# labicon/dp-ilqr

Hardware: AMD Instinct MI355X
Metric: ilqr_subproblems_per_sec (higher is better)
Workload: dtype f64; 1 GPU; cfg2: batches of 1024 independent 5-agent DoubleIntDynamics4D iLQR sub-problems per GPU per step, T=50, scripts/analysis.py scenario distribution, tol=1e-3, n_lqr_iter=50; 2468 steps = 2527232 distinct seeds per GPU, window of 6144 in flight; 1 repetition(s) of the job on disjoint seeds, the median is reported; batch_per_gpu=1024, window=6144, n_x=20, n_u=10, horizon=50, parallelism=single GPU

## Files before the change

### dpilqr_amd/csrc/admit_order.hpp

```cpp
#pragma once
#include <cstdint>

#if defined(__HIPCC__)
#include <hip/hip_runtime.h>
#define DPILQR_HD __host__ __device__
#else
#define DPILQR_HD
#endif

namespace dpilqr {

enum CostOrder : int { kOrderOff = 0, kOrderSpread = 1, kOrderGrouped = 2 };
constexpr int kDefaultCostOrder = kOrderSpread;

constexpr int kOrderMinLive = 1024;
constexpr int kOrderClasses = 64;

struct SweepDeal {
    int n, n_cus, waves, per_layer, layers, rounds, lo, extra;
    DPILQR_HD SweepDeal(int n_, int n_cus_, int waves_) : n(n_), n_cus(n_cus_), waves(waves_) {
        const int lpr = waves / 4;
        per_layer = 4 * n_cus;
        layers = (n + per_layer - 1) / per_layer;
        rounds = (layers + lpr - 1) / lpr;
        lo = rounds > 0 ? layers / rounds : 0;
        extra = rounds > 0 ? layers - lo * rounds : 0;
    }
    DPILQR_HD int layers_of(int round) const { return lo + (round < extra ? 1 : 0); }
    DPILQR_HD int first_layer(int round) const { return round * lo + (round < extra ? round : extra); }
    DPILQR_HD int round_of_layer(int layer) const {
        const int head = extra * (lo + 1);
        return layer < head ? layer / (lo + 1) : extra + (layer - head) / (lo > 0 ? lo : 1);
    }
    DPILQR_HD int slot(int round, int cu, int wave) const {
        if (round >= rounds || wave >= 4 * layers_of(round)) return -1;
        const int s = (first_layer(round) + (wave >> 2)) * per_layer + (wave & 3) * n_cus + cu;
        return s < n ? s : -1;
    }
};

DPILQR_HD inline int order_position(int rank, const SweepDeal& D, int order) {
    if (order != kOrderGrouped) return rank;
    const int round = D.round_of_layer(rank / D.per_layer);
    const int f = D.first_layer(round), m = D.layers_of(round);
    const int q = rank - f * D.per_layer;
    int base = 4 * m, e = 0;
    if (round == D.rounds - 1) {
        const int rem = D.n - (D.layers - 1) * D.per_layer;
        base = 4 * (m - 1) + rem / D.n_cus;
        e = rem % D.n_cus;
    }
    int cu, w;
    if (q < e * (base + 1)) { cu = q / (base + 1); w = q - cu * (base + 1); }
    else { const int q2 = q - e * (base + 1), per = base > 0 ? base : 1; cu = e + q2 / per; w = q2 - (cu - e) * per; }
    return (f + (w >> 2)) * D.per_layer + (w & 3) * D.n_cus + cu;
}

DPILQR_HD inline int order_class(int key, int T) {
    const int top = T + 1;
    const int c = top < kOrderClasses ? key : (int)((int64_t)key * (kOrderClasses - 1) / top);
    return c < 0 ? 0 : (c > kOrderClasses - 1 ? kOrderClasses - 1 : c);
}

#if defined(__HIPCC__) && defined(DPILQR_ADMIT_ORDER_KERNELS)

constexpr int kKeyStagedAgents = 5;
__global__ void __launch_bounds__(256) k_cost_keys(const double* __restrict__ X, const double* __restrict__ radius, int64_t radius_bstride,
                                                   const int32_t* __restrict__ list, const int32_t* __restrict__ count, int B, int T, int k,
                                                   int min_live, int32_t* __restrict__ key) {
    __shared__ double2 sP[4][64 * kKeyStagedAgents];
    const int n = count ? *count : B;
    if (n <= min_live) return;
    const int wave = (int)threadIdx.x >> 6, lane = threadIdx.x & 63;
    const int pos = (int)blockIdx.x * 4 + wave;
    if (pos >= n) return;
    const int b = list ? list[pos] : pos;
    if (b < 0 || b >= B) return;
    const double r = radius[(int64_t)b * radius_bstride];
    const double lim = r * r * (1.0 + 1e-12);
    const int nx = 4 * k;
    const double* Xb = X + (int64_t)b * (T + 1) * nx;
    const bool staged = k <= kKeyStagedAgents;
    int cnt = 0;
    for (int t0 = 0; t0 <= T; t0 += 64) {
        const int rows = min(64, T + 1 - t0);
        bool near = false;
        if (staged) {
            const double2* src = reinterpret_cast<const double2*>(Xb + (int64_t)t0 * nx);
            for (int e = lane; e < rows * k; e += 64) sP[wave][e] = src[2 * e];
            __builtin_amdgcn_wave_barrier();
            asm volatile("" ::: "memory");
            if (lane < rows) {
                double2 p[kKeyStagedAgents];
#pragma unroll
                for (int i = 0; i < kKeyStagedAgents; ++i) p[i] = sP[wave][lane * k + min(i, k - 1)];
#pragma unroll
                for (int i = 0; i < kKeyStagedAgents; ++i)
#pragma unroll
                    for (int j = i + 1; j < kKeyStagedAgents; ++j) {
                        const double ddx = p[i].x - p[j].x, ddy = p[i].y - p[j].y;
                        const double s2 = ddx * ddx + ddy * ddy;
                        near = near || (j < k && !(s2 > lim));
                    }
            }
            __builtin_amdgcn_wave_barrier();
            asm volatile("" ::: "memory");
        } else if (lane < rows) {
            const double* row = Xb + (int64_t)(t0 + lane) * nx;
            for (int i = 0; i < k; ++i)
                for (int j = i + 1; j < k; ++j) {
                    const double ddx = row[4 * i] - row[4 * j], ddy = row[4 * i + 1] - row[4 * j + 1];
                    const double s2 = ddx * ddx + ddy * ddy;
                    near = near || !(s2 > lim);
                }
        }
        cnt += __popcll(__builtin_amdgcn_ballot_w64(near));
    }
    if (lane == 0) key[pos] = cnt;
}

__global__ void __launch_bounds__(1024) k_order_list(const int32_t* __restrict__ src, int32_t* __restrict__ dst, const int32_t* __restrict__ count,
                                                     const int32_t* __restrict__ key, int T, int n_cus, int waves, int order, int min_live) {
    static_assert(kOrderClasses == 64, "the prefix sums below are one wavefront's, a bin per lane");
    __shared__ int hist[kOrderClasses], cursor[kOrderClasses];
    const int n = *count;
    if (n <= min_live || order == kOrderOff) {
        for (int i = threadIdx.x; i < n; i += blockDim.x) dst[i] = src[i];
        return;
    }
    if (threadIdx.x < kOrderClasses) hist[threadIdx.x] = 0;
    __syncthreads();
    for (int i = threadIdx.x; i < n; i += blockDim.x) atomicAdd(&hist[kOrderClasses - 1 - order_class(key[i], T)], 1);
    __syncthreads();
    if (threadIdx.x < kOrderClasses) {
        const int own = hist[threadIdx.x];
        int run = own;
        for (int off = 1; off < kOrderClasses; off <<= 1) {
            const int below = __shfl_up(run, off);
            if ((int)threadIdx.x >= off) run += below;
        }
        cursor[threadIdx.x] = run - own;
    }
    __syncthreads();
    const SweepDeal deal(n, n_cus, waves);
    for (int i = threadIdx.x; i < n; i += blockDim.x) {
        const int rank = atomicAdd(&cursor[kOrderClasses - 1 - order_class(key[i], T)], 1);
        const int pos = order_position(rank, deal, order);
        if (pos >= 0 && pos < n) dst[pos] = src[i];
    }
}

// ... 4 lines not shown
```

### dpilqr_amd/csrc/dpilqr_hip.hip

```cpp
#include <hip/hip_runtime.h>

#include <cstdarg>
#include <cstdio>
#include <algorithm>
#include <cstdlib>
#include <cstring>
#include <new>
#include <vector>

#include "dpilqr_hip.h"
#include "admit_order.hpp"
#include "launch.hpp"
#include "models.hpp"
#include "tiles.hpp"

namespace dpilqr {

static thread_local char g_err[512] = "";

int32_t fail(int32_t code, const char* fmt, ...) {
    va_list ap;
    va_start(ap, fmt);
    vsnprintf(g_err, sizeof(g_err), fmt, ap);
    va_end(ap);
// ... 368 lines not shown
    };

    int32_t* admitted_dev = counts + kCountRing;
    S.fault = counts + kCountRing + 1;
    static const bool no_static = route_flag("DPILQR_TILES_NO_STATIC");
    const int um = hint_model(D);
    const bool fused = sh.fused;
    const bool static_part = !fused && !sh.big && !no_static && D.R_bstride == 0 &&
                             (um == kDoubleInt4D || um == kDoubleInt6D || um == kHumanLin6D);
    if (!resume) {
        double a[DPILQR_N_ALPHA];
        alpha_table(a);
        const int init_n = D.B > kCountRing + 2 ? D.B : kCountRing + 2;
        hipLaunchKernelGGL(k_init_state, dim3((init_n + 255) / 256), dim3(256), 0, st, D.B, S.mu, S.delta, status, n_bwd, n_fwd,
                           singular, counts, kCountRing + 2, alphas, a[0], a[1], a[2], a[3], a[4], a[5], a[6], a[7], a[8], a[9]);
        HIP_TRY(hipGetLastError());
        prof.begin(3, -1, st);
        rc = Passes<R>::forward(D, kModeRollout, x0, X, U, nullptr, nullptr, nullptr, 1, nullptr, nullptr, S.J_star, S, nullptr,
                                nullptr, D.B, st);
        if (rc) return bail(rc);
        prof.end(st);
        hipLaunchKernelGGL(k_copy_f64, dim3((D.B + 255) / 256), dim3(256), 0, st, D.B, S.J_star, S.J_last);
        if (n_lqr_iter > 0) {
            if (!fused && hipMemsetAsync(tiles, 0, W.K - W.tiles, st) != hipSuccess) return bail(fail(DPILQR_EHIP, "hipMemsetAsync failed"));
            if (static_part) {
                if constexpr (sizeof(R) == 8) {
                    if ((rc = launch_make_tiles(D, X, U, tiles, nullptr, nullptr, Wn, true, false, st))) return bail(rc);
                }
            }
        }
    }

    static const int order_route = route_flag("DPILQR_NO_COST_ORDER") ? (int)kOrderOff : route_int("DPILQR_COST_ORDER", kDefaultCostOrder);
    const int order = (sizeof(R) == 8 && fused && (order_route == kOrderSpread || order_route == kOrderGrouped)) ? order_route : (int)kOrderOff;
    int32_t* keys = reinterpret_cast<int32_t*>(ws + W.Xc);
    int surv = 0;
    size_t n_iterations = 0;
    auto enqueue_iteration = [&](int it, int upper) -> int32_t {
        int32_t* cur = lists + (size_t)surv * Wn;
        int32_t* other = lists + (size_t)(surv ^ 1) * Wn;
        int32_t* cur_n = counts + (it % kCountRing);
        int32_t* nxt_n = counts + ((it + 1) % kCountRing);
        int32_t* mail = solver ? solver->dev + kMailWords * (it % kMailRing) : nullptr;
        hipLaunchKernelGGL(k_admit, dim3(1), dim3(256), 0, st, cur, cur_n, nxt_n, admitted_dev, D.B, Wn, mail,
                           (solver && solver->progress) ? 1 : 0, t_admit, S.fault);
        if (solver) HIP_TRY(hipEventRecord(solver->ev[it % kMailRing], st));
        int32_t r = DPILQR_OK;
        const int order_waves = order ? fused_sweep_tier(D, upper) : 0;
        if (order_waves > 0) {
            if constexpr (sizeof(R) == 8) {
                if ((r = launch_cost_keys(D, X, cur, cur_n, upper, kOrderMinLive, keys, st))) return r;
                if ((r = launch_order_list(cur, other, cur_n, keys, D.T, device_cus(), order_waves, order, kOrderMinLive, st))) return r;
            }
            S.next_items = cur;
            cur = other;
        } else {
            S.next_items = other;
            surv ^= 1;
        }
        S.next_count = nxt_n;
        if (fused) {
            if constexpr (sizeof(R) == 8) {
                prof.begin(1, it, st);
                if ((r = launch_riccati_fused(D, X, U, S.mu, K, d, singular, cur, cur_n, upper, S.gains_by_item, st))) return r;
                prof.end(st, g_sweep_waves);
            }
        } else if (!sh.big) {
            if constexpr (sizeof(R) == 8) {
                prof.begin(0, it, st);
                if ((r = launch_make_tiles(D, X, U, tiles, cur, cur_n, upper, true, static_part, st))) return r;
                prof.end(st);
                prof.begin(1, it, st);
                if ((r = launch_riccati(D.B, D.T, n, m, tiles, S.mu, K, d, singular, cur, cur_n, upper, S.gains_by_item, D.n_s,
                                        D.n_c, st)))
                    return r;
                prof.end(st, g_sweep_waves);
            }
        } else {
            prof.begin(1, it, st);
            if ((r = Passes<R>::sweep_big(D, X, U, S.mu, K, d, singular, cur, cur_n, upper, S.gains_by_item, tiles, st))) return r;
            prof.end(st, 0);
        }
        prof.begin(2, it, st);
        if ((r = Passes<R>::forward(D, kModeLineSearch, nullptr, X, U, K, d, alphas, DPILQR_N_ALPHA, Xc, Uc, nullptr, S, cur, cur_n,
// ... 416 lines not shown
                               float* K_out, float* d_out, void* stream) {
    if (!solver) {
        const int32_t rc = default_solver(&solver);
        if (rc) return rc;
    }
    return solve_impl<float>(solver, desc, x0, U, n_lqr_iter, tol, t_kill, window, workspace, workspace_bytes, X, J, status, n_bwd,
                             n_fwd, trace, K_out, d_out, 0, 0, as_stream(stream));
}
int32_t dpilqr_solve_enqueue(const dpilqr_batch_desc* desc, const double* x0, double* U, int32_t n_lqr_iter, double tol,
                             double t_kill, int32_t window, void* workspace, int64_t workspace_bytes, double* X, double* J, int32_t* status,
                             int32_t* n_bwd, int32_t* n_fwd, double* trace, double* K_out, double* d_out,
                             int32_t n_global_iter, int32_t resume, void* stream) {
    return solve_impl<double>(nullptr, desc, x0, U, n_lqr_iter, tol, t_kill, window, workspace, workspace_bytes, X, J, status, n_bwd,
                              n_fwd, trace, K_out, d_out, n_global_iter, resume, as_stream(stream));
}
int64_t dpilqr_solve_iterations_bound(const dpilqr_batch_desc* desc, int32_t window, int32_t n_lqr_iter) {
    if (!desc || desc->B < 0 || n_lqr_iter < 0) return fail(DPILQR_EINVAL, "solve_iterations_bound: bad argument");
    const int64_t W = window_of(*desc, window);
    return ((int64_t)desc->B + W - 1) / W * n_lqr_iter + 1;
}

int32_t dpilqr_debug_stamps(void* buf) {
    int32_t rc = set_stamp_buffer_riccati(buf);
    return rc ? rc : set_stamp_buffer_forward(buf);
}

int32_t dpilqr_cost_keys(const dpilqr_batch_desc* desc, const double* X, const int32_t* items, const int32_t* n_items, int32_t* keys,
                         void* stream) {
    int32_t rc = check_desc(desc);
    if (rc) return rc;
    if (desc->n_s != 4) return fail(DPILQR_EUNSUPPORTED, "cost_keys: n_s=%d, the keys are defined for the four-state family", desc->n_s);
    if (desc->B == 0) return DPILQR_OK;
    if (!X || !keys || ((items == nullptr) != (n_items == nullptr))) return fail(DPILQR_EINVAL, "cost_keys: NULL pointer");
    return launch_cost_keys(*desc, X, items, n_items, desc->B, -1, keys, as_stream(stream));
}

int32_t dpilqr_order_list(const int32_t* items, const int32_t* n_items, const int32_t* keys, int32_t T, int32_t n_cus, int32_t waves,
                          int32_t order, int32_t* out, void* stream) {
    if (!items || !n_items || !keys || !out) return fail(DPILQR_EINVAL, "order_list: NULL pointer");
    if (T < 1 || n_cus < 1 || (waves != 4 && waves != 8 && waves != 12) || (order != kOrderSpread && order != kOrderGrouped))
        return fail(DPILQR_EINVAL, "order_list: T=%d n_cus=%d waves=%d order=%d", T, n_cus, waves, order);
    return launch_order_list(items, out, n_items, keys, T, n_cus, waves, order, -1, as_stream(stream));
}

int32_t dpilqr_order_position(int32_t rank, int32_t n, int32_t n_cus, int32_t waves, int32_t order) {
    if (n < 1 || rank < 0 || rank >= n || n_cus < 1 || (waves != 4 && waves != 8 && waves != 12) ||
        (order != kOrderSpread && order != kOrderGrouped))
        return fail(DPILQR_EINVAL, "order_position: rank=%d n=%d n_cus=%d waves=%d order=%d", rank, n, n_cus, waves, order);
    return order_position(rank, SweepDeal(n, n_cus, waves), order);
}

int32_t dpilqr_profile_enable(dpilqr_solver* solver, int32_t enable) {
    Profiler& g_prof = solver ? solver->prof : g_default_solver.prof;
    const int32_t prev = g_prof.on ? 1 : 0;
    g_prof.on = (enable & 1) != 0;
    g_prof.mask = (enable >> 1) & 0xF ? (enable >> 1) & 0xF : 0xF;
    return prev;
}

int32_t dpilqr_profile_read(dpilqr_solver* solver, double ms[4], int64_t launches[4], int64_t items[4], int32_t reset) {
    if (!ms || !launches || !items) return fail(DPILQR_EINVAL, "profile_read: NULL pointer");
    Profiler& g_prof = solver ? solver->prof : g_default_solver.prof;
    for (int c = 0; c < 4; ++c) {
        ms[c] = g_prof.ms[c]; launches[c] = g_prof.launches[c]; items[c] = g_prof.items[c];
        if (reset) { g_prof.ms[c] = 0; g_prof.launches[c] = 0; g_prof.items[c] = 0; }
    }
    return DPILQR_OK;
// ... 21 lines not shown
```

### dpilqr_amd/csrc/launch.hpp

```cpp
#pragma once
#include <hip/hip_runtime.h>

#include <cstdint>
#include <cstdlib>

#include "dpilqr_hip.h"
#include "solve_state.hpp"

namespace dpilqr {

int32_t fail(int32_t code, const char* fmt, ...);
const char* last_error();

#define HIP_TRY(expr)                                                                                 \
    do {                                                                                              \
        hipError_t e_ = (expr);                                                                       \
        if (e_ != hipSuccess) return ::dpilqr::fail(DPILQR_EHIP, "%s failed: %s", #expr, hipGetErrorString(e_)); \
    } while (0)

constexpr int kMaxLds = 160 * 1024;

template <typename Kern>
inline int32_t allow_lds(Kern kern, size_t bytes) {
    if (bytes > (size_t)kMaxLds) return fail(DPILQR_EUNSUPPORTED, "needs %zu B of LDS per workgroup (> %d)", bytes, kMaxLds);
// ... 78 lines not shown
    return grid_items <= cus ? grid_items : (grid_items + cus * wv - 1) / (cus * wv) * cus;
}
inline int sweep_max_waves() { static const int v = route_int("DPILQR_MFMA_WAVES", 12); return v; }
template <typename Kern, typename... Args>
int32_t launch_sweep_kernel(Kern kern, int wv, int threads, size_t lds, int grid_items, int cus, hipStream_t st, const Args&... args) {
    const int32_t rc = allow_lds(kern, lds);
    if (rc) return rc;
    hipLaunchKernelGGL(kern, dim3(sweep_grid(grid_items, cus, wv)), dim3(threads), lds, st, args...);
    HIP_TRY(hipGetLastError());
    g_sweep_waves = wv;
    return DPILQR_OK;
}
template <typename T> struct same_type { using type = T; };
template <typename Kern, typename... Args>
int32_t launch_wave_sweep(Kern k4, typename same_type<Kern>::type k8, typename same_type<Kern>::type k12, size_t lds_per_wave,
                          int grid_items, int cus, hipStream_t st, const Args&... args) {
    const int wv = sweep_waves(grid_items, sweep_max_waves(), lds_per_wave, k12 != nullptr);
    return launch_sweep_kernel(wv == 12 ? k12 : (wv == 8 ? k8 : k4), wv, 64 * wv, lds_per_wave * wv, grid_items, cus, st, args...);
}
int32_t launch_riccati_team(const dpilqr_batch_desc& D, const double* X, const double* U, const double* mu, double* K, double* d,
                            int32_t* singular, const int32_t* items, const int32_t* n_items, int grid_items, int gains_by_item,
                            hipStream_t st);

int32_t launch_riccati_inprod(const dpilqr_batch_desc& D, const double* X, const double* U, const double* mu, double* K, double* d,
                              int32_t* singular, const int32_t* items, const int32_t* n_items, int grid_items, int gains_by_item,
                              hipStream_t st);

int32_t launch_riccati_bike(const dpilqr_batch_desc& D, const double* X, const double* U, const double* mu, double* K, double* d,
                            int32_t* singular, const int32_t* items, const int32_t* n_items, int grid_items, int gains_by_item,
                            hipStream_t st);

int fused_sweep_tier(const dpilqr_batch_desc& D, int grid_items);
int32_t launch_cost_keys(const dpilqr_batch_desc& D, const double* X, const int32_t* list, const int32_t* count, int grid_items,
                         int min_live, int32_t* key, hipStream_t st);
int32_t launch_order_list(const int32_t* src, int32_t* dst, const int32_t* count, const int32_t* key, int T, int cus, int waves,
                          int order, int min_live, hipStream_t st);

int32_t launch_linesearch_team(const dpilqr_batch_desc& D, double* X, double* U, const double* K, const double* d,
                               const double* alphas, double* Xc, double* Uc, const SolveState& S, const int32_t* items,
                               const int32_t* n_items, int grid_items, hipStream_t st);

int32_t launch_forward(const dpilqr_batch_desc& D, int mode, const double* x0, double* X, double* U, const double* K,
                       const double* d, const double* alphas, int ngrp, double* Xc, double* Uc, double* Jc,
                       const SolveState& S, const int32_t* items, const int32_t* n_items, int grid_items,
                       hipStream_t st);
int32_t set_stamp_buffer_forward(void* device_buffer);
int32_t launch_model_op(int op, int32_t n, int32_t ns, const int32_t* model, const double* x, const double* u, double dt,
                        double* o1, double* o2, hipStream_t st);
int32_t launch_cost_eval(const dpilqr_batch_desc& D, int32_t n_pts, const double* x, const double* u, int32_t terminal,
                         double* cost, hipStream_t st);
int32_t launch_pairwise_graph(int32_t S, int32_t N, int32_t k, int32_t n_s, const double* X, const double* radius,
                              int32_t* adj, hipStream_t st);


int32_t launch_policy_rollout(const dpilqr_batch_desc& D, const double* X, const double* U, const double* K, int32_t n_samples,
                              const double* x0s, const double* W, const double* u_lim, double* Xs, double* Us, double* J,
                              double* min_sep, double* goal_dist, hipStream_t st);
int32_t launch_policy_rollout_dec(const dpilqr_batch_desc& D, const double* X, const double* U_ff, const double* Kc, int32_t kc_max,
                                  const uint64_t* nbr_bits, int32_t n_samples, const double* x0s, const double* W, const double* u_lim,
                                  double* Xs, double* Us, double* J, double* min_sep, double* goal_dist, hipStream_t st);

int32_t launch_policy_rollout_dec_team(const dpilqr_batch_desc& D, const double* X, const double* U_ff, const double* Kc, int32_t kc_max,
                                       const uint64_t* nbr_bits, int32_t n_samples, const double* x0s, const double* W,
                                       const double* u_lim, double* Xs, double* Us, double* J, double* min_sep, double* goal_dist,
                                       hipStream_t st);

int32_t launch_policy_advance(const dpilqr_batch_desc& D, const double* X, const double* U, const double* K, int32_t kc_max,
// ... 38 lines not shown
```

### dpilqr_amd/csrc/riccati_mfma.hpp

```cpp
#pragma once
#include <hip/hip_runtime.h>

#include <type_traits>

#include "tiles.hpp"
#include "wave_util.hpp"

namespace dpilqr {

typedef double v4d __attribute__((ext_vector_type(4)));

template <int N, int M, int FUSED = 0, bool HELP = false>
struct MfmaCfg {
    static constexpr int NM = N + M;
    static constexpr int NP = N + 1;
    static constexpr int MK = round_up(M, 4);
    static constexpr int LAB = round_up(NM, 2);
    static constexpr int LT = LAB;
    static constexpr int LP = round_up(NP, 2);
    static constexpr int LQ = LP;
    static constexpr int LG = round_up(M + NP, 2);
    static constexpr int LK = LP;
    static constexpr int LM = N;
    static constexpr int KROWS = MK + 2;
// ... 182 lines not shown
#pragma unroll
                for (int q = 0; q < 3; ++q)
                    if (r0 + q < M) { tm[q] = v[r0 + q] * ninv; asm volatile("" : "+v"(tm[q])); }
                if (r0 + 2 >= M) asm volatile("s_nop 1");
#pragma unroll
                for (int q = 0; q < 3; ++q)
                    if (r0 + q < M) { v[r0 + q] = fmac_row_nn(v[r0 + q], tm[q], v[kk], kk); asm volatile("" : "+v"(v[r0 + q])); }
            }
            }
        } else {
#pragma unroll
            for (int r = kk + 1; r < M; ++r) {
                const double l = readlane_f64(v[r], kk) * inv;
                v[r] = fma(-l, v[kk], v[r]);
            }
        }
    }
#pragma unroll
    for (int r = 0; r < M; ++r) v_io[r] = v[r];
}

__device__ __forceinline__ void wave_barrier_all() { asm volatile("s_waitcnt lgkmcnt(0)\n\ts_barrier" ::: "memory"); }

template <bool ON>
__device__ __forceinline__ int phase_lane(int lane) {
    if constexpr (ON) asm volatile("" : "+v"(lane));
    return lane;
}

struct FusedArgs {
    dpilqr_batch_desc D;
    const double* X;
    const double* U;
};

template <int N, int M, int WAVES, int NS, int NC, int FUSED, bool PAD = false, bool HELP = false, int PNS = 0>
__device__ __forceinline__ void riccati_mfma_sweep(
    int B, int T, const double* __restrict__ tiles, const double* __restrict__ mu_arr, double* __restrict__ Kout,
    double* __restrict__ dout, int32_t* __restrict__ singular, const int32_t* __restrict__ items,
    const int32_t* __restrict__ n_items, int gains_by_item, int n_cus, FusedArgs F, int n_rec = N, int m_rec = M) {
    using C = MfmaCfg<N, M, FUSED, HELP>;
    static_assert(!FUSED || (NS == 4 && NC == 2), "the fused variants are written for the four-state family's blocks");
    static_assert(!HELP || (FUSED != 0 && WAVES == 4), "the helper wavefront serves the fused forms at one item per SIMD");
    static_assert(!PAD || (NS == 0 && FUSED == 0), "padding while loading is written for the dense record-fed form");
    static_assert(PNS == 0 || (NS == 0 && FUSED == 0 && !HELP), "in-sweep production builds on the dense form (padded, or of the exact size: n_rec = N, m_rec = M)");
    constexpr bool INP = PNS > 0;
    using IC = InprodCfg<N, M, PNS>;
    constexpr bool FGEN = (FUSED == 2);
    constexpr int NM = C::NM, NP = C::NP, MK = C::MK, LAB = C::LAB, LT = C::LT, LP = C::LP, LQ = C::LQ, LG = C::LG;
    constexpr int LK = C::LK, LM = C::LM, T_NM = C::T_NM, T_NP = C::T_NP, T_N = C::T_N, T_M = C::T_M;
    const int wave_all = threadIdx.x >> 6;
    const bool helper = HELP && wave_all >= 4;
    const int wave = HELP ? (wave_all & 3) : wave_all;
    const int n = n_items ? *n_items : B;
    constexpr int LPR = WAVES / 4;
    const int per_layer = 4 * n_cus;
    const int layers = (n + per_layer - 1) / per_layer;
    const int rounds = (layers + LPR - 1) / LPR;
    const int round = (int)blockIdx.x / n_cus, cu = (int)blockIdx.x - round * n_cus;
    if (round >= rounds) return;
    const int lo = layers / rounds, extra = layers - lo * rounds;
    const int my_layers = lo + (round < extra ? 1 : 0);
    const int first_layer = round * lo + min(round, extra);
    if (wave >= 4 * my_layers) return;
    const int slot = (first_layer + (wave >> 2)) * per_layer + (wave & 3) * n_cus + cu;
    if (slot >= n) return;
// ... 51 lines not shown
            wave_barrier_all();
            {
                t_cur = T - 1;
#include "riccati_mfma_lane.inc"
                fused_prefetch(T - 1);
            }
            for (int t = T - 1; t >= 0; --t) {
                t_cur = t;
#include "riccati_mfma_lane.inc"
                __builtin_amdgcn_s_waitcnt(0x0F70);
                fused_step_data(t, nullptr);
                if (lane == 0) sFflag[0] = f_prox ? 1.0 : 0.0;
                if (t > 0) fused_prefetch(t - 1);
                if constexpr (C::TEAM_TAIL) {
                    if (t < T - 1) {
                        wave_barrier_all();
                        constexpr int IT = 1;
#include "riccati_mfma_team_tail.inc"
                    }
                }
                wave_barrier_all();
            }
            if constexpr (C::TEAM_TAIL) {
                t_cur = 0;
#include "riccati_mfma_lane.inc"
                wave_barrier_all();
                constexpr int IT = 1;
#include "riccati_mfma_team_tail.inc"
                wave_barrier_all();
            }
            return;
        }
    }
    if constexpr (FUSED) {
        const ItemParams IP = item_params(F.D, b);
        constexpr int FKA_ = C::F_KA;
        const int ag_ = min(lane0 / LPA, KA - 1), sub2_ = min(lane0 - (lane0 / LPA) * LPA, (NM - 1) / RPL);
#pragma unroll
        for (int r = 0; r < RPL; ++r) {
#pragma unroll
            for (int c = 0; c < NSC; ++c) lvc[r][c] = 0.0;
            lv_h[r] = -1; lv_neg[r] = false;
            const int ip = min(RPL * sub2_ + r, NM - 1);
            if (ip < N) {
                const int ar = ip >> 2, li = ip & 3;
                if (ar == ag_) {
                    const double* Qa = IP.Q + (FGEN ? 16 * ag_ : 0);
#pragma unroll
                    for (int c = 0; c < NS; ++c) lvc[r][c] = F.D.w_ref * (Qa[li * 4 + c] + Qa[c * 4 + li]);
                }
                if (FKA_ > 1 && li < 2) {
                    lv_neg[r] = ar != ag_;
                    lv_h[r] = (ar == ag_) ? (C::oFD - C::oFH) + ag_ * 4 + li * 2
                                          : ((ar < ag_) ? pair_index(ar, ag_, FKA_) : pair_index(ag_, ar, FKA_)) * 4 + li * 2;
                }
            } else {
                const int a = ip - N;
                if ((a >> 1) == ag_) {
                    const double* Ra = IP.R + (FGEN ? 4 * ag_ : 0);
                    lvc[r][NS] = F.D.w_ref * (Ra[(a & 1) * 2] + Ra[a & 1]);
                    lvc[r][NS + 1] = F.D.w_ref * (Ra[(a & 1) * 2 + 1] + Ra[2 + (a & 1)]);
                }
            }
        }
    }
#include "riccati_mfma_inprod.inc"
    {
    const int lane = lane0;
    for (int e = lane; e < C::total + IC::total; e += 64) lds[e] = 0.0;
    DPILQR_LDS_FENCE();
    if constexpr (INP) {
        inp_constants();
        inp_prefetch(T);
        inp_produce(T, true);
        for (int e = lane; e < N * N; e += 64) {
            const int i = e / N, j = e - i * N;
            sP[i * LP + j] = sLxx[e];
        }
        for (int i = lane; i < N; i += 64) sP[i * LP + N] = sLxu[i];
        DPILQR_LDS_FENCE();
        inp_lxx_blocks(false, true);
        inp_prefetch(T - 1);
    } else if constexpr (!FUSED) {
        const double* rec = base + (int64_t)T * L.stride;
        for (int e = lane; e < N * N; e += 64) {
            const int i = e / N, j = e - i * N;
            if constexpr (PAD) {
                const double val = rec[L.oLxx + min(i, n_rec - 1) * n_rec + min(j, n_rec - 1)];
                sP[i * LP + j] = (i < n_rec && j < n_rec) ? val : 0.0;
            } else {
            sP[i * LP + j] = rec[L.oLxx + e];
            }
        }
        for (int i = lane; i < N; i += 64) {
            const double val = rec[L.oLx + (PAD ? min(i, n_rec - 1) : i)];
            sP[i * LP + N] = (!PAD || i < n_rec) ? val : 0.0;
        }
    }
// ... 22 lines not shown
        fused_step_data(T, IP.Qf);
        for (int e = lane; e < N * N; e += 64) {
            const int i = e / N, j = e - i * N, ai = i >> 2, li = i & 3, aj = j >> 2, lj = j & 3;
            double val = 0.0;
            if (ai == aj) {
                const double* Qfa = IP.Qf + (FGEN ? 16 * ai : 0);
                val = F.D.w_ref * (Qfa[li * 4 + lj] + Qfa[lj * 4 + li]);
            }
            if (FKA > 1 && li < 2 && lj < 2 && f_prox) {
                double acc = 0.0;
                if (ai == aj) acc = sFD[ai * 4 + li * 2 + lj];
                else acc += -sFH[((ai < aj) ? pair_index(ai, aj, FKA) : pair_index(aj, ai, FKA)) * 4 + li * 2 + lj];
                val += F.D.w_prox * acc;
            }
            sP[i * LP + j] = val;
        }
        for (int j = lane; j < N; j += 64) sP[j * LP + N] = sFL[j];
        DPILQR_LDS_FENCE();
        if constexpr (!HELP) fused_prefetch(T - 1);
    } else if constexpr (INP) {
    } else {
    prefetch_ab(T - 1);
    if constexpr (BD) {
        prefetch_bd_x(T - 1);
        if constexpr (!LATE_L) prefetch_bd_l(T - 1);
    } else {
        prefetch_lxu(T - 1);
        prefetch_l(T - 1);
    }
    }
    __builtin_amdgcn_s_waitcnt(0x0F70);
    }

#ifdef DPILQR_PHASE_STAMPS
    unsigned long long ph[8] = {0, 0, 0, 0, 0, 0, 0, 0}, ph_t = __builtin_amdgcn_s_memtime();
#define MPHASE(i) { asm volatile("s_waitcnt lgkmcnt(0)" ::: "memory"); const unsigned long long now_ = __builtin_amdgcn_s_memtime(); ph[i] += now_ - ph_t; ph_t = now_; }
#elif defined(DPILQR_PHASE_MARKS)
#define MPHASE(i) asm volatile("; ==== end of phase " #i);
#else
#define MPHASE(i)
#endif
    for (int t = T - 1; t >= 0; --t) {
        const int tn = t > 0 ? t - 1 : 0;
        t_cur = t;
        {
        const int lane = phase_lane<REMAT>(lane0);
#include "riccati_mfma_lane.inc"
        if constexpr (HELP) {
            wave_barrier_all();
            f_prox = __builtin_amdgcn_readfirstlane((int)(sFflag[0] != 0.0)) != 0;
        } else if constexpr (FUSED) {
            fused_step_data(t, nullptr);
            fused_prefetch(tn);
        } else if constexpr (INP) {
            inp_produce(t, false);
            inp_prefetch(tn);
        } else {
#pragma unroll
        for (int q = 0; q < C::AB_ROUNDS; ++q) *reinterpret_cast<v2d*>(ab_dst[q]) = nAB[q];
        DPILQR_LDS_FENCE();
        if constexpr (LATE_L) prefetch_bd_l(t);
        prefetch_ab(tn);
        }
        MPHASE(0)

        __builtin_amdgcn_s_setprio(1);
        if constexpr (FUSED) {
            const double fdt = F.D.dt;
            double acc[NSC][CPL], pr[NS][CPL];
#pragma unroll
            for (int l = 0; l < NS; ++l) {
                const v2d v = *reinterpret_cast<const v2d*>(bP + l * LP);
                pr[l][0] = v.x; pr[l][1] = v.y;
            }
            double fa[4] = {0.0, 0.0, 0.0, 0.0};
// ... 427 lines not shown
```

### dpilqr_amd/csrc/tu_order.hip

```cpp
#include <hip/hip_runtime.h>

#define DPILQR_ADMIT_ORDER_KERNELS
#include "admit_order.hpp"
#include "launch.hpp"
#include "riccati_mfma.hpp"

namespace dpilqr {

int fused_sweep_tier(const dpilqr_batch_desc& D, int grid_items) {
    if (!fused_wavefront_sweep_applies(D) || grid_items <= kOrderMinLive) return 0;
    const int n = D.k * D.n_s, m = D.k * D.n_c;
#define DPILQR_TIER(NN, MM) \
    if (n == NN && m == MM) return sweep_waves(grid_items, sweep_max_waves(), sizeof(double) * MfmaCfg<NN, MM, true>::total, true);
    DPILQR_TIER(4, 2) DPILQR_TIER(8, 4) DPILQR_TIER(12, 6) DPILQR_TIER(16, 8) DPILQR_TIER(20, 10)
#undef DPILQR_TIER
    return 0;
}

int32_t launch_cost_keys(const dpilqr_batch_desc& D, const double* X, const int32_t* list, const int32_t* count, int grid_items,
                         int min_live, int32_t* key, hipStream_t st) {
    if (grid_items <= 0) return DPILQR_OK;
    hipLaunchKernelGGL(k_cost_keys, dim3((grid_items + 3) / 4), dim3(256), 0, st, X, D.radius, D.radius_bstride, list, count, D.B, D.T,
                       D.k, min_live, key);
    HIP_TRY(hipGetLastError());
    return DPILQR_OK;
}

int32_t launch_order_list(const int32_t* src, int32_t* dst, const int32_t* count, const int32_t* key, int T, int cus, int waves,
                          int order, int min_live, hipStream_t st) {
    hipLaunchKernelGGL(k_order_list, dim3(1), dim3(1024), 0, st, src, dst, count, key, T, cus, waves, order, min_live);
    HIP_TRY(hipGetLastError());
    return DPILQR_OK;
}

}
```

### dpilqr_amd/csrc/tu_riccati.hip

```cpp
#include <hip/hip_runtime.h>

#include <cstdlib>
#include <cstring>

#include "launch.hpp"
#include "riccati.hpp"
#include "riccati_mfma.hpp"
#include "riccati_wg.hpp"

namespace dpilqr {

static int riccati_threads(int n) { return n <= 24 ? 64 : (n <= 36 ? 128 : 256); }

#define DPILQR_WAVE_SIZES(X) X(4, 2) X(8, 4) X(12, 6) X(16, 8) X(20, 10)

#define DPILQR_WG_SIZES(X)                                                                                      \
    X(6, 4, 2) X(7, 4, 2) X(8, 4, 2) X(9, 4, 2) X(10, 4, 2) X(11, 4, 2) X(12, 4, 2) X(13, 4, 2) X(14, 4, 2) X(15, 4, 2) \
    X(2, 6, 3) X(3, 6, 3) X(4, 6, 3) X(5, 6, 3) X(6, 6, 3) X(7, 6, 3) X(8, 6, 3) X(9, 6, 3) X(10, 6, 3)
#define DPILQR_WG_RECORD_SIZES(X) \
    X(2, 12, 4) X(3, 12, 4) X(4, 12, 4) X(5, 12, 4) X(1, 6, 3) X(1, 12, 4) X(2, 3, 2) X(4, 3, 2) X(6, 3, 2)

thread_local int g_sweep_waves = 0;

template <bool FUSED, typename... Args>
// ... 62 lines not shown
        DPILQR_TRY_PAD(24, 12)
#undef DPILQR_TRY_PAD
    }
    static const bool no_wg = route_flag("DPILQR_RICCATI_NO_WG");
    if (!generic && !no_wg && block_ns > 0) {
        const int32_t rc_w = launch_riccati_wg<false>(n, m, block_ns, block_nc, grid_items, st, B, T, tiles, mu, K, d, singular,
                                                      items, n_items, gains_by_item, FusedArgs{});
        if (rc_w != DPILQR_EUNSUPPORTED) return rc_w;
    }
    const size_t lds = riccati_lds_bytes(n, m);
    int32_t rc = allow_lds(k_riccati_generic, lds);
    if (rc) return rc;
    hipLaunchKernelGGL(k_riccati_generic, dim3(grid_items), dim3(riccati_threads(n)), lds, st, B, T, n, m, tiles, mu, K,
                       d, singular, items, n_items, gains_by_item);
    HIP_TRY(hipGetLastError());
    return DPILQR_OK;
}

int32_t launch_riccati_fused(const dpilqr_batch_desc& D, const double* X, const double* U, const double* mu, double* K,
                             double* d, int32_t* singular, const int32_t* items, const int32_t* n_items, int grid_items,
                             int gains_by_item, hipStream_t st) {
    g_sweep_waves = 0;
    if (grid_items <= 0) return DPILQR_OK;
    const int n = D.k * D.n_s, m = D.k * D.n_c;
    {
        const int32_t rc_ip = launch_riccati_inprod(D, X, U, mu, K, d, singular, items, n_items, grid_items, gains_by_item, st);
        if (rc_ip != DPILQR_EUNSUPPORTED) return rc_ip;
    }
    if (grid_items <= 1024 && sweep_max_waves() >= 4 && (fused_wavefront_sweep_applies(D) || fused_wavefront_general_applies(D))) {
        const int32_t rc_team = launch_riccati_team(D, X, U, mu, K, d, singular, items, n_items, grid_items, gains_by_item, st);
        if (rc_team != DPILQR_EUNSUPPORTED) return rc_team;
    }
    const int cus = device_cus();
#define DPILQR_TRY_FUSED(NN, MM)                                                                                   \
    if (n == NN && m == MM)                                                                                        \
        return launch_wave_sweep(k_riccati_mfma<NN, MM, 4, 4, 2, true>, k_riccati_mfma<NN, MM, 8, 4, 2, true>,     \
                                 k_riccati_mfma<NN, MM, 12, 4, 2, true>, sizeof(double) * MfmaCfg<NN, MM, true>::total, \
                                 grid_items, cus, st, D.B, D.T, nullptr, mu, K, d, singular, items, n_items, gains_by_item, \
                                 cus, FusedArgs{D, X, U});
    if (fused_wavefront_sweep_applies(D)) {
        DPILQR_WAVE_SIZES(DPILQR_TRY_FUSED)
    }
#undef DPILQR_TRY_FUSED
#define DPILQR_TRY_FUSED2(NN, MM)                                                                                  \
    if (n == NN && m == MM)                                                                                        \
        return launch_wave_sweep(k_riccati_mfma_general<NN, MM, 4>, k_riccati_mfma_general<NN, MM, 8>, nullptr,    \
                                 sizeof(double) * MfmaCfg<NN, MM, 2>::total, grid_items, cus, st, D.B, D.T, mu, K, d, \
                                 singular, items, n_items, gains_by_item, cus, FusedArgs{D, X, U});
    if (fused_wavefront_general_applies(D)) {
        DPILQR_WAVE_SIZES(DPILQR_TRY_FUSED2)
    }
#undef DPILQR_TRY_FUSED2
    if (fused_workgroup_sweep_applies(D))
        return launch_riccati_wg<true>(n, m, D.n_s, D.n_c, grid_items, st, D.B, D.T, nullptr, mu, K, d, singular, items, n_items,
                                       gains_by_item, FusedArgs{D, X, U});
    return DPILQR_EUNSUPPORTED;
}

int32_t set_stamp_buffer_riccati(void* buf) {
    void* p = buf;
    HIP_TRY(hipMemcpyToSymbol(HIP_SYMBOL(g_stamp_buf), &p, sizeof(p)));
    return DPILQR_OK;
}

}
```

Baseline: 1.080 million subproblems/s.

## Add decoupled per-agent Riccati prologue for trailing steps without proximity coupling

Adds a prologue to the fused MFMA Riccati sweep. While no proximity cost is active, it runs the backward recursion for the trailing timesteps with a cheap per-agent decoupled 4x2 block update and writes the gains directly. It drops to the full coupled MFMA loop at the first step with coupling or a failed conditioning check. The cost-order key also changes from a near-step count to the index of the last dense step, which matches the new per-item cost. The price is extra code, LDS traffic and divergence in the kernel, plus a different ordering heuristic.

```diff
diff --git a/dpilqr_amd/csrc/admit_order.hpp b/dpilqr_amd/csrc/admit_order.hpp
--- a/dpilqr_amd/csrc/admit_order.hpp
+++ b/dpilqr_amd/csrc/admit_order.hpp
@@ -12,6 +12,8 @@
 
 enum CostOrder : int { kOrderOff = 0, kOrderSpread = 1, kOrderGrouped = 2 };
 constexpr int kDefaultCostOrder = kOrderSpread;
+enum CostKey : int { kKeyNearCount = 0, kKeyDenseSteps = 1 };
+constexpr int kDefaultCostKey = kKeyDenseSteps;
 
 constexpr int kOrderMinLive = 1024;
 constexpr int kOrderClasses = 64;
@@ -67,7 +69,7 @@
 constexpr int kKeyStagedAgents = 5;
 __global__ void __launch_bounds__(256) k_cost_keys(const double* __restrict__ X, const double* __restrict__ radius, int64_t radius_bstride,
                                                    const int32_t* __restrict__ list, const int32_t* __restrict__ count, int B, int T, int k,
-                                                   int min_live, int32_t* __restrict__ key) {
+                                                   int min_live, int32_t* __restrict__ key, int32_t* __restrict__ key_dense) {
     __shared__ double2 sP[4][64 * kKeyStagedAgents];
     const int n = count ? *count : B;
     if (n <= min_live) return;
@@ -81,7 +83,7 @@
     const int nx = 4 * k;
     const double* Xb = X + (int64_t)b * (T + 1) * nx;
     const bool staged = k <= kKeyStagedAgents;
-    int cnt = 0;
+    int cnt = 0, dense = 0;
     for (int t0 = 0; t0 <= T; t0 += 64) {
         const int rows = min(64, T + 1 - t0);
         bool near = false;
@@ -114,9 +116,14 @@
                     near = near || !(s2 > lim);
                 }
         }
-        cnt += __popcll(__builtin_amdgcn_ballot_w64(near));
+        const unsigned long long mask = __builtin_amdgcn_ballot_w64(near);
+        cnt += __popcll(mask);
+        if (mask) dense = t0 + 64 - __clzll(mask);
     }
-    if (lane == 0) key[pos] = cnt;
+    if (lane == 0) {
+        if (key) key[pos] = cnt;
+        if (key_dense) key_dense[pos] = dense;
+    }
 }
 
 __global__ void __launch_bounds__(1024) k_order_list(const int32_t* __restrict__ src, int32_t* __restrict__ dst, const int32_t* __restrict__ count,
diff --git a/dpilqr_amd/csrc/dpilqr_hip.hip b/dpilqr_amd/csrc/dpilqr_hip.hip
--- a/dpilqr_amd/csrc/dpilqr_hip.hip
+++ b/dpilqr_amd/csrc/dpilqr_hip.hip
@@ -424,6 +424,7 @@
     }
 
     static const int order_route = route_flag("DPILQR_NO_COST_ORDER") ? (int)kOrderOff : route_int("DPILQR_COST_ORDER", kDefaultCostOrder);
+    static const bool dense_key = !route_flag("DPILQR_NO_DECOUPLED") && route_int("DPILQR_COST_KEY", kDefaultCostKey) == (int)kKeyDenseSteps;
     const int order = (sizeof(R) == 8 && fused && (order_route == kOrderSpread || order_route == kOrderGrouped)) ? order_route : (int)kOrderOff;
     int32_t* keys = reinterpret_cast<int32_t*>(ws + W.Xc);
     int surv = 0;
@@ -441,7 +442,7 @@
         const int order_waves = order ? fused_sweep_tier(D, upper) : 0;
         if (order_waves > 0) {
             if constexpr (sizeof(R) == 8) {
-                if ((r = launch_cost_keys(D, X, cur, cur_n, upper, kOrderMinLive, keys, st))) return r;
+                if ((r = launch_cost_keys(D, X, cur, cur_n, upper, kOrderMinLive, dense_key ? nullptr : keys, dense_key ? keys : nullptr, st))) return r;
                 if ((r = launch_order_list(cur, other, cur_n, keys, D.T, device_cus(), order_waves, order, kOrderMinLive, st))) return r;
             }
             S.next_items = cur;
@@ -924,7 +925,8 @@
     if (desc->n_s != 4) return fail(DPILQR_EUNSUPPORTED, "cost_keys: n_s=%d, the keys are defined for the four-state family", desc->n_s);
     if (desc->B == 0) return DPILQR_OK;
     if (!X || !keys || ((items == nullptr) != (n_items == nullptr))) return fail(DPILQR_EINVAL, "cost_keys: NULL pointer");
-    return launch_cost_keys(*desc, X, items, n_items, desc->B, -1, keys, as_stream(stream));
+    static const bool second = route_flag("DPILQR_KEYS_DENSE_STEPS");
+    return launch_cost_keys(*desc, X, items, n_items, desc->B, -1, second ? nullptr : keys, second ? keys : nullptr, as_stream(stream));
 }
 
 int32_t dpilqr_order_list(const int32_t* items, const int32_t* n_items, const int32_t* keys, int32_t T, int32_t n_cus, int32_t waves,
diff --git a/dpilqr_amd/csrc/launch.hpp b/dpilqr_amd/csrc/launch.hpp
--- a/dpilqr_amd/csrc/launch.hpp
+++ b/dpilqr_amd/csrc/launch.hpp
@@ -134,7 +134,7 @@
 
 int fused_sweep_tier(const dpilqr_batch_desc& D, int grid_items);
 int32_t launch_cost_keys(const dpilqr_batch_desc& D, const double* X, const int32_t* list, const int32_t* count, int grid_items,
-                         int min_live, int32_t* key, hipStream_t st);
+                         int min_live, int32_t* key, int32_t* key_dense, hipStream_t st);
 int32_t launch_order_list(const int32_t* src, int32_t* dst, const int32_t* count, const int32_t* key, int T, int cus, int waves,
                           int order, int min_live, hipStream_t st);
 
diff --git a/dpilqr_amd/csrc/riccati_mfma.hpp b/dpilqr_amd/csrc/riccati_mfma.hpp
--- a/dpilqr_amd/csrc/riccati_mfma.hpp
+++ b/dpilqr_amd/csrc/riccati_mfma.hpp
@@ -238,6 +238,7 @@
     dpilqr_batch_desc D;
     const double* X;
     const double* U;
+    int no_decoupled = 0;
 };
 
 template <int N, int M, int WAVES, int NS, int NC, int FUSED, bool PAD = false, bool HELP = false, int PNS = 0>
@@ -355,38 +356,6 @@
             return;
         }
     }
-    if constexpr (FUSED) {
-        const ItemParams IP = item_params(F.D, b);
-        constexpr int FKA_ = C::F_KA;
-        const int ag_ = min(lane0 / LPA, KA - 1), sub2_ = min(lane0 - (lane0 / LPA) * LPA, (NM - 1) / RPL);
-#pragma unroll
-        for (int r = 0; r < RPL; ++r) {
-#pragma unroll
-            for (int c = 0; c < NSC; ++c) lvc[r][c] = 0.0;
-            lv_h[r] = -1; lv_neg[r] = false;
-            const int ip = min(RPL * sub2_ + r, NM - 1);
-            if (ip < N) {
-                const int ar = ip >> 2, li = ip & 3;
-                if (ar == ag_) {
-                    const double* Qa = IP.Q + (FGEN ? 16 * ag_ : 0);
-#pragma unroll
-                    for (int c = 0; c < NS; ++c) lvc[r][c] = F.D.w_ref * (Qa[li * 4 + c] + Qa[c * 4 + li]);
-                }
-                if (FKA_ > 1 && li < 2) {
-                    lv_neg[r] = ar != ag_;
-                    lv_h[r] = (ar == ag_) ? (C::oFD - C::oFH) + ag_ * 4 + li * 2
-                                          : ((ar < ag_) ? pair_index(ar, ag_, FKA_) : pair_index(ag_, ar, FKA_)) * 4 + li * 2;
-                }
-            } else {
-                const int a = ip - N;
-                if ((a >> 1) == ag_) {
-                    const double* Ra = IP.R + (FGEN ? 4 * ag_ : 0);
-                    lvc[r][NS] = F.D.w_ref * (Ra[(a & 1) * 2] + Ra[a & 1]);
-                    lvc[r][NS + 1] = F.D.w_ref * (Ra[(a & 1) * 2 + 1] + Ra[2 + (a & 1)]);
-                }
-            }
-        }
-    }
 #include "riccati_mfma_inprod.inc"
     {
     const int lane = lane0;
@@ -475,6 +444,200 @@
     __builtin_amdgcn_s_waitcnt(0x0F70);
     }
 
+    int t_first = T - 1;
+    if constexpr (FUSED == 1 && !HELP) {
+        if (!F.no_decoupled && !f_prox) {
+            const int lane = lane0;
+            static_assert(32 * KA <= C::szG, "the prologue's exchange area must fit the G region");
+            const ItemParams IP = item_params(F.D, b);
+            const int da = min(lane >> 3, KA - 1), dc = min(lane & 7, 4);
+            const bool dst = dc < 4;
+            const int dcol = dst ? 4 * da + dc : N;
+            const double fdt = F.D.dt, wref = F.D.w_ref;
+            double* sX = sG + 32 * da;
+            double Pc[4];
+#pragma unroll
+            for (int l = 0; l < 4; ++l) Pc[l] = sP[(4 * da + l) * LP + dcol];
+            const int cq = dc & 3, cr = dc & 1;
+            const double inf_ = __builtin_inf();
+            double chk0 = fabs(mu) + fabs(fdt);
+#pragma unroll
+            for (int l = 0; l < 4; ++l) chk0 = chk0 + fabs(Pc[l]);
+            if (__builtin_amdgcn_ballot_w64(!(chk0 < inf_)) == 0ull) {
+                DPILQR_LDS_FENCE();
+                for (int e = lane; e < C::szR2; e += 64) sT[e] = 0.0;
+                static_assert(20 <= N * LQ, "the prologue's constants must fit the Q_xx region");
+                if (lane < 16) sQ[lane] = wref * (IP.Q[(lane & 3) * 4 + (lane >> 2)] + IP.Q[(lane >> 2) * 4 + (lane & 3)]);
+                else if (lane < 20) sQ[lane] = wref * (IP.R[(lane & 1) * 2 + ((lane >> 1) & 1)] + IP.R[((lane >> 1) & 1) * 2 + (lane & 1)]);
+                DPILQR_LDS_FENCE();
+                int t = T - 1;
+                for (; t >= 0; --t) {
+                    t_cur = t;
+                    const int lane = phase_lane<REMAT>(lane0);
+#include "riccati_mfma_lane.inc"
+                    fused_step_data(t, nullptr);
+                    if (f_prox) break;
+                    fused_prefetch(t > 0 ? t - 1 : 0);
+                    double tt[6];
+                    tt[0] = Pc[0];
+                    tt[1] = Pc[1];
+                    tt[2] = fdt * Pc[0] + Pc[2];
+                    tt[3] = fdt * Pc[1] + Pc[3];
+                    tt[4] = fdt * Pc[2];
+                    tt[5] = fdt * Pc[3];
+                    tt[4] = fma(mu, (dst && dc == 2) ? fdt : 0.0, tt[4]);
+                    tt[5] = fma(mu, (dst && dc == 3) ? fdt : 0.0, tt[5]);
+                    if (dc < 2) {
+#pragma unroll
+                        for (int r = 0; r < 6; ++r) sX[2 * r + dc] = tt[r];
+                    }
+                    DPILQR_LDS_FENCE();
+                    double qc[4], gc[2], quu[2];
+                    {
+                        double tu[6], lx[6], lq[4], lr[2];
+                        {
+                            const v2d q0 = *reinterpret_cast<const v2d*>(sQ + 4 * cq), q1 = *reinterpret_cast<const v2d*>(sQ + 4 * cq + 2),
+                                      r0 = *reinterpret_cast<const v2d*>(sQ + 16 + 2 * cr);
+                            lq[0] = q0.x; lq[1] = q0.y; lq[2] = q1.x; lq[3] = q1.y; lr[0] = r0.x; lr[1] = r0.y;
+                        }
+#pragma unroll
+                        for (int r = 0; r < 6; ++r) tu[r] = sX[2 * r + cr];
+#pragma unroll
+                        for (int r = 0; r < 4; ++r) lx[r] = sFL[4 * da + r];
+                        lx[4] = sFL[N + 2 * da]; lx[5] = sFL[N + 2 * da + 1];
+#pragma unroll
+                        for (int r = 0; r < 6; ++r) {
+                            const double o = (dc < 2) ? tt[r] : tu[r] * fdt + tt[r];
+                            const double qv = (r < 4 ? lq[r] : 0.0) + o;
+                            const double v = dst ? qv : lx[r] + tt[r];
+                            if (r < 4) qc[r] = v; else gc[r - 4] = v;
+                        }
+#pragma unroll
+                        for (int a = 0; a < 2; ++a) quu[a] = lr[a] + tt[4 + a] * fdt;
+                    }
+                    DPILQR_LDS_FENCE();
+                    if (dc == 2 || dc == 3) { sX[12 + cr] = quu[0]; sX[14 + cr] = quu[1]; }
+                    DPILQR_LDS_FENCE();
+                    const double u00 = sX[12], u01 = sX[13], u10 = sX[14], u11 = sX[15];
+                    bool ok;
+                    {
+                        const double cs0 = (0.0 + fabs(u00)) + fabs(u10), cs1 = (0.0 + fabs(u01)) + fabs(u11);
+                        const double dg0 = fabs(u00), dg1 = fabs(u11);
+                        ok = (dg0 * (1.0 - 0x1p-20) > cs0 - dg0) && (dg1 * (1.0 - 0x1p-20) > cs1 - dg1);
+                    }
+                    double inv0 = __builtin_amdgcn_rcp(u00);
+                    inv0 = fma(fma(-u00, inv0, 1.0), inv0, inv0);
+                    inv0 = fma(fma(-u00, inv0, 1.0), inv0, inv0);
+                    const double tm = u10 * (-inv0);
+                    const double w11 = fma(tm, u01, u11), g1 = fma(tm, gc[0], gc[1]);
+                    double inv1 = __builtin_amdgcn_rcp(w11);
+                    inv1 = fma(fma(-w11, inv1, 1.0), inv1, inv1);
+                    inv1 = fma(fma(-w11, inv1, 1.0), inv1, inv1);
+                    double kc[2];
+                    kc[1] = -(g1 * inv1);
+                    kc[0] = -(fma(u01, kc[1], gc[0]) * inv0);
+                    ok = ok && u00 != 0.0 && w11 != 0.0;
+                    const double t30 = fma(u10, kc[1], fma(u00, kc[0], 0.0)), t31 = fma(u11, kc[1], fma(u01, kc[0], 0.0));
+                    DPILQR_LDS_FENCE();
+                    if (dst) {
+                        *reinterpret_cast<v2d*>(sX + 6 * dc) = v2d{t30, t31};
+                        *reinterpret_cast<v2d*>(sX + 6 * dc + 2) = v2d{kc[0], kc[1]};
+                        *reinterpret_cast<v2d*>(sX + 6 * dc + 4) = v2d{gc[0], gc[1]};
+                    }
+                    DPILQR_LDS_FENCE();
+                    double vc[4];
+#pragma unroll
+                    for (int i = 0; i < 4; ++i) {
+                        const v2d e0 = *reinterpret_cast<const v2d*>(sX + 6 * i), e1 = *reinterpret_cast<const v2d*>(sX + 6 * i + 2),
+                                  e2 = *reinterpret_cast<const v2d*>(sX + 6 * i + 4);
+                        const double a1 = fma(e0.y, kc[1], fma(e0.x, kc[0], 0.0));
+                        const double a2 = fma(e1.y, gc[1], fma(e1.x, gc[0], 0.0));
+                        const double a2t = fma(kc[1], e2.y, fma(kc[0], e2.x, 0.0));
+                        vc[i] = ((qc[i] + a1) + a2) + a2t;
+                    }
+                    DPILQR_LDS_FENCE();
+                    if (dst) {
+#pragma unroll
+                        for (int i = 0; i < 4; ++i) sX[4 * i + dc] = vc[i];
+                    }
+                    DPILQR_LDS_FENCE();
+                    double pn[4];
+                    {
+                        const v2d w0 = *reinterpret_cast<const v2d*>(sX + 4 * cq), w1 = *reinterpret_cast<const v2d*>(sX + 4 * cq + 2);
+                        pn[0] = dst ? 0.5 * (vc[0] + w0.x) : vc[0];
+                        pn[1] = dst ? 0.5 * (vc[1] + w0.y) : vc[1];
+                        pn[2] = dst ? 0.5 * (vc[2] + w1.x) : vc[2];
+                        pn[3] = dst ? 0.5 * (vc[3] + w1.y) : vc[3];
+                    }
+                    DPILQR_LDS_FENCE();
+                    double chk = fabs(u00) + fabs(u01);
+                    chk = chk + fabs(u10); chk = chk + fabs(u11); chk = chk + fabs(w11); chk = chk + fabs(inv0); chk = chk + fabs(inv1);
+                    chk = chk + fabs(gc[0]); chk = chk + fabs(gc[1]); chk = chk + fabs(g1); chk = chk + fabs(kc[0]); chk = chk + fabs(kc[1]);
+                    chk = chk + fabs(t30); chk = chk + fabs(t31);
+#pragma unroll
+                    for (int i = 0; i < 4; ++i) chk = chk + fabs(pn[i]);
+                    ok = ok && chk < inf_;
+                    if (__builtin_amdgcn_ballot_w64(!ok) != 0ull) {
+                        fused_prefetch(t);
+                        break;
+                    }
+#pragma unroll
+                    for (int l = 0; l < 4; ++l) Pc[l] = pn[l];
+                    sK[(2 * da) * LK + dcol] = kc[0];
+                    sK[(2 * da + 1) * LK + dcol] = kc[1];
+                    DPILQR_LDS_FENCE();
+                    double* Kt = Kout + (gslot * T + t) * M * N;
+                    double* dt_ = dout + (gslot * T + t) * M;
+#pragma unroll
+                    for (int q = 0; q < K_ROUNDS; ++q) store_v2d_nt(Kt + k_out[q], *reinterpret_cast<const v2d*>(sK + k_in[q]));
+                    store_f64_nt(dt_ + d_idx, sK[d_idx * LK + N]);
+                    DPILQR_LDS_FENCE();
+                }
+                t_first = t;
+                for (int e = lane; e < 32 * KA; e += 64) sG[e] = 0.0;
+                if (lane < 20) sQ[lane] = 0.0;
+                for (int e = lane; e < C::szR2; e += 64) sT[e] = 0.0;
+                DPILQR_LDS_FENCE();
+#pragma unroll
+                for (int l = 0; l < 4; ++l) sP[(4 * da + l) * LP + dcol] = Pc[l];
+                DPILQR_LDS_FENCE();
+            }
+        }
+    }
+
+    if constexpr (FUSED) {
+        const ItemParams IP = item_params(F.D, b);
+        constexpr int FKA_ = C::F_KA;
+        const int ag_ = min(lane0 / LPA, KA - 1), sub2_ = min(lane0 - (lane0 / LPA) * LPA, (NM - 1) / RPL);
+#pragma unroll
+        for (int r = 0; r < RPL; ++r) {
+#pragma unroll
+            for (int c = 0; c < NSC; ++c) lvc[r][c] = 0.0;
+            lv_h[r] = -1; lv_neg[r] = false;
+            const int ip = min(RPL * sub2_ + r, NM - 1);
+            if (ip < N) {
+                const int ar = ip >> 2, li = ip & 3;
+                if (ar == ag_) {
+                    const double* Qa = IP.Q + (FGEN ? 16 * ag_ : 0);
+#pragma unroll
+                    for (int c = 0; c < NS; ++c) lvc[r][c] = F.D.w_ref * (Qa[li * 4 + c] + Qa[c * 4 + li]);
+                }
+                if (FKA_ > 1 && li < 2) {
+                    lv_neg[r] = ar != ag_;
+                    lv_h[r] = (ar == ag_) ? (C::oFD - C::oFH) + ag_ * 4 + li * 2
+                                          : ((ar < ag_) ? pair_index(ar, ag_, FKA_) : pair_index(ag_, ar, FKA_)) * 4 + li * 2;
+                }
+            } else {
+                const int a = ip - N;
+                if ((a >> 1) == ag_) {
+                    const double* Ra = IP.R + (FGEN ? 4 * ag_ : 0);
+                    lvc[r][NS] = F.D.w_ref * (Ra[(a & 1) * 2] + Ra[a & 1]);
+                    lvc[r][NS + 1] = F.D.w_ref * (Ra[(a & 1) * 2 + 1] + Ra[2 + (a & 1)]);
+                }
+            }
+        }
+    }
+
 #ifdef DPILQR_PHASE_STAMPS
     unsigned long long ph[8] = {0, 0, 0, 0, 0, 0, 0, 0}, ph_t = __builtin_amdgcn_s_memtime();
 #define MPHASE(i) { asm volatile("s_waitcnt lgkmcnt(0)" ::: "memory"); const unsigned long long now_ = __builtin_amdgcn_s_memtime(); ph[i] += now_ - ph_t; ph_t = now_; }
@@ -483,7 +646,7 @@
 #else
 #define MPHASE(i)
 #endif
-    for (int t = T - 1; t >= 0; --t) {
+    for (int t = t_first; t >= 0; --t) {
         const int tn = t > 0 ? t - 1 : 0;
         t_cur = t;
         {
diff --git a/dpilqr_amd/csrc/tu_order.hip b/dpilqr_amd/csrc/tu_order.hip
--- a/dpilqr_amd/csrc/tu_order.hip
+++ b/dpilqr_amd/csrc/tu_order.hip
@@ -18,10 +18,10 @@
 }
 
 int32_t launch_cost_keys(const dpilqr_batch_desc& D, const double* X, const int32_t* list, const int32_t* count, int grid_items,
-                         int min_live, int32_t* key, hipStream_t st) {
+                         int min_live, int32_t* key, int32_t* key_dense, hipStream_t st) {
     if (grid_items <= 0) return DPILQR_OK;
     hipLaunchKernelGGL(k_cost_keys, dim3((grid_items + 3) / 4), dim3(256), 0, st, X, D.radius, D.radius_bstride, list, count, D.B, D.T,
-                       D.k, min_live, key);
+                       D.k, min_live, key, key_dense);
     HIP_TRY(hipGetLastError());
     return DPILQR_OK;
 }
diff --git a/dpilqr_amd/csrc/tu_riccati.hip b/dpilqr_amd/csrc/tu_riccati.hip
--- a/dpilqr_amd/csrc/tu_riccati.hip
+++ b/dpilqr_amd/csrc/tu_riccati.hip
@@ -118,12 +118,13 @@
         if (rc_team != DPILQR_EUNSUPPORTED) return rc_team;
     }
     const int cus = device_cus();
+    static const bool no_dec = route_flag("DPILQR_NO_DECOUPLED");
 #define DPILQR_TRY_FUSED(NN, MM)                                                                                   \
     if (n == NN && m == MM)                                                                                        \
         return launch_wave_sweep(k_riccati_mfma<NN, MM, 4, 4, 2, true>, k_riccati_mfma<NN, MM, 8, 4, 2, true>,     \
                                  k_riccati_mfma<NN, MM, 12, 4, 2, true>, sizeof(double) * MfmaCfg<NN, MM, true>::total, \
                                  grid_items, cus, st, D.B, D.T, nullptr, mu, K, d, singular, items, n_items, gains_by_item, \
-                                 cus, FusedArgs{D, X, U});
+                                 cus, FusedArgs{D, X, U, no_dec ? 1 : 0});
     if (fused_wavefront_sweep_applies(D)) {
         DPILQR_WAVE_SIZES(DPILQR_TRY_FUSED)
     }
```

Result: faster. 1.308 million subproblems/s (median of 6 runs) (+21.1%).
